# wangkenpu/rsrgan

Hardware: AMD Instinct MI355X
Metric: GAN train frames/sec (G+D step), 257-dim LPS->40-dim MFCC (higher is better)
Workload: dtype f32

## Files before the change

rsrgan_amd/csrc/capi.cpp:

```cpp
#include <cstring>
#include <exception>
#include <new>
#include <vector>

#include "model.h"

using namespace rsr;

struct rsrgan_handle_s { Model m; };

#define CHECK_H(h)                                                    \
  if (!(h)) { set_error("null handle"); return RSRGAN_ERR_INVALID; }

template <class F>
static int guard(const char* what, F&& body) {
  try {
    return body();
  } catch (const std::bad_alloc&) {
    set_error("%s: out of host memory", what);
  } catch (const std::exception& e) {
    set_error("%s: %s", what, e.what());
  } catch (...) {
    set_error("%s: unknown C++ exception", what);
  }
// ... 398 lines not shown
    float ms = 0.f;
    if (hipEventElapsedTime(&ms, m.prof_ev[2 * i], m.prof_ev[2 * i + 1]) != hipSuccess) { set_error("hipEventElapsedTime failed"); return RSRGAN_ERR_HIP; }
    us += 1e3 * ms;
  }
  *launches = m.prof_n; *total_us = us; *alg_flops = m.prof_flops;
  return RSRGAN_OK;
}
int rsrgan_profile_read_kind(rsrgan_handle h, int32_t kind, int32_t* launches, double* total_us, double* alg_flops) {
  CHECK_H(h);
  if (kind == 0) return rsrgan_profile_read(h, launches, total_us, alg_flops);
  Model& m = h->m;
  if (kind == 3 && launches && total_us && alg_flops) {
    *launches = m.prof_fdt_n; *total_us = 0.0; *alg_flops = 0.0;
    return RSRGAN_OK;
  }
  if (kind >= 4 && kind <= 8 && launches && total_us && alg_flops) {
    *launches = m.prof_cnt[kind]; *total_us = 0.0; *alg_flops = 0.0;
    return RSRGAN_OK;
  }
  if ((kind != 1 && kind != 2) || !launches || !total_us || !alg_flops) { set_error("profile_read_kind: bad argument"); return RSRGAN_ERR_INVALID; }
  std::vector<hipEvent_t>& ev = kind == 1 ? m.prof_gp_ev : m.prof_gb_ev;
  const int n = kind == 1 ? m.prof_gp_n : m.prof_gb_n;
  double us = 0.0;
  for (int i = 0; i < n; ++i) {
    if (hipEventSynchronize(ev[2 * i + 1]) != hipSuccess) { set_error("hipEventSynchronize failed"); return RSRGAN_ERR_HIP; }
    float ms = 0.f;
    if (hipEventElapsedTime(&ms, ev[2 * i], ev[2 * i + 1]) != hipSuccess) { set_error("hipEventElapsedTime failed"); return RSRGAN_ERR_HIP; }
    us += 1e3 * ms;
  }
  *launches = n; *total_us = us; *alg_flops = kind == 1 ? m.prof_gp_flops : m.prof_gb_flops;
  return RSRGAN_OK;
// ... 50 lines not shown
```

rsrgan_amd/csrc/gpersist.hip:

```cpp
#include <type_traits>

#include "kernels.h"

namespace rsr {

typedef float f32x4 __attribute__((ext_vector_type(4)));
typedef unsigned u32x4 __attribute__((ext_vector_type(4)));
typedef __attribute__((address_space(1))) unsigned gu32;
#include "dpersist_dev.h"

constexpr int GP_NR = GP_ROWS / 16;
constexpr int GP_WAVES = 12;
static_assert(GP_NR == 2, "chunk index = 2 * k-block + row tile");
constexpr int GP_NKB = 18;
constexpr int GP_KBW = 5;
constexpr int GP_SLOT = 1024;
constexpr unsigned GP_SENT = 0xFFFFFFFFu;
#ifndef GP_R1_STEPS
#define GP_R1_STEPS 3
#endif
constexpr int GP_R1 = GP_R1_STEPS;
constexpr int GP_NCH = GP_NKB * GP_NR;
constexpr unsigned GP_SC1 = 16u;
constexpr unsigned GP_VOL = 1u << 31;
// ... 851 lines not shown
      const unsigned g1 = gen + 1u;
      __hip_atomic_store(ctl + DP_CTL_GEN, g1 >= (1u << 21) ? 1u : g1, __ATOMIC_RELAXED, __HIP_MEMORY_SCOPE_AGENT);
    }
  }
}

#ifndef GP_XR_STEPS
#define GP_XR_STEPS 6
#endif
constexpr int GP_XR = GP_XR_STEPS;

template <int NT>
struct GpLdsB {
  unsigned cnt_p[GP_NR], cnt_h[GP_NR], cnt_m[GP_NR], cnt_g[GP_NR], cnt_z[GP_NR], cnt_f[GP_NR], cnt_q[GP_NR], cnt_d[GP_NR], dead, pad_[3];
  float peep[4 * NT][4];
  float car[4][2][GP_NR][64][2];
  float gs[2][GP_NR][2][64][4];
  float st[4][GP_ROWS][4 * NT];
  float pfs[GP_NR][5][16][4 * NT];
  float wpb[GP_NKB][16][4];
  float dzB[GP_NR][NT][64][4];
  float pd[4][GP_NR][NT][64];
  float wpa[GP_NKB][64][4];
  float mB[GP_NR][GP_NKB][64][4];
  float kl[8][NT][64][4];
};

__device__ __forceinline__ bool gp_poll(const GpBuf& b, unsigned so, bool son, gu32* err) {
  const unsigned long long t0 = __builtin_amdgcn_s_memrealtime();
  for (unsigned polls = 0;; ++polls) {
// ... 260 lines not shown
#pragma unroll
    for (int r = 0; r < NR; ++r)
#pragma unroll
      for (int sl = 0; sl < 2; ++sl)
        *reinterpret_cast<float2*>(&S.car[w][sl][r][lane][0]) = make_float2(L.c[((size_t)T * N + row0 + 16 * r + lr) * H + min(cell0 + 4 * (w + 4 * sl) + q, H - 1)], 0.f);
    float* const carw = &S.car[w][0][0][lane][0];
    const float* const pfc = &S.pfs[0][0][lr][4 * w + q];
    const float* const mbw = &S.mB[0][w][lane][0];
    const float* const wpw = &S.wpa[w][lane][0];
    const float* const wpv = &S.wpb[w][4 * q + (lr >> 2)][0];
    float* const pdw = &S.pd[w][0][0][lane];
    const float* const pdc = &S.pd[0][0][w][lane];
    const float* const pwc = &S.peep[4 * w + q][0];
    float* const dzw = &S.dzB[0][w][lane][0];
    float* const stc = &S.st[0][lr][4 * w + q];
    for (int s = 0; s < T; ++s) {
      const int t = T - 1 - s;
#ifdef GP_TRACE
      if (s == 0 && w == 0 && lane == 0) gp_tr[0][22] = (unsigned)__builtin_amdgcn_s_memtime();
#endif
#pragma unroll
      for (int r = 0; r < NR; ++r) {
        if (r >= nrt) continue;
        GPTSR(6 * r + 0);
        if (!gp_wait(cnt + C_M + r, 2u * ((unsigned)s + 1u), dead)) return;
        GPTSR(6 * r + 1);

        {
          f32x4 d0 = {0.f, 0.f, 0.f, 0.f}, d1 = {0.f, 0.f, 0.f, 0.f};
          __builtin_amdgcn_s_setprio(2);
// ... 33 lines not shown
            const float gi = pq[0], gj = pq[16 * CW], gf = pq[2 * 16 * CW], go = pq[3 * 16 * CW], cp = pq[4 * 16 * CW];
            const float2 cv = *reinterpret_cast<const float2*>(carw + (sl * NR + r) * 128);
            const float cc = cv.x, dcv = cv.y;
            const float tc = gp_tanh(cc);
            const float dao = dh * tc * go * (1.f - go);
            const float dcn = dcv + dh * go * (1.f - tc * tc) + dao * pw[2];
            const float daf = dcn * cp * gf * (1.f - gf);
            const float dai = dcn * gj * gi * (1.f - gi);
            const float dj = dcn * gi * (1.f - gj * gj);
            const float dcx = live ? dcn * gf + dai * pw[0] + daf * pw[1] : dcv;
            *reinterpret_cast<float2*>(carw + (sl * NR + r) * 128) = make_float2(cp, dcx);
            const f32x4 dz = {live ? dai : 0.f, live ? dj : 0.f, live ? daf : 0.f, live ? dao : 0.f};
            *reinterpret_cast<f32x4*>(dzw + (r * NT + 4 * sl) * 256) = dz;
            float* const d = stc + r * 16 * CW + sl * 16;
            d[0 * GP_ROWS * CW] = dz[0]; d[1 * GP_ROWS * CW] = dz[1]; d[2 * GP_ROWS * CW] = dz[2]; d[3 * GP_ROWS * CW] = dz[3];
          }
        }
        asm volatile("s_waitcnt vmcnt(0)" ::: "memory");
        gp_signal(cnt + C_H + r, lane);
        GPTSR(6 * r + 4);
        if (!gp_wait(cnt + C_H + r, 4u * ((unsigned)s + 1u), dead)) return;
        if (t > 0) { product(r, (int)((c1 + (unsigned)s) % GP_R1), ((c1 + (unsigned)s) / GP_R1) & 1u); gp_signal(cnt + C_Q + r, lane); }
        GPTSR(6 * r + 5);
        int ln = lane;
        asm volatile("" : "+v"(ln));
#pragma unroll
        for (int it = 0; it < (4 * 16 * NT + 255) / 256; ++it) {
          const int e = it * 256 + w * 64 + ln;
          const int cq = e % NT, pr = e / NT, row = 16 * r + (pr & 15), k = min(pr >> 4, 3);
          const float4 v = *reinterpret_cast<const float4*>(&S.st[k][row][4 * cq]);
          float* dst = L.gates + ((size_t)t * N + row0 + row) * H4 + k * H + cell0 + 4 * cq;
#ifdef GP_ABL2
          if (GP_ABL2 & 16) continue;
#endif
          if (e < 4 * 16 * NT && cell0 + 4 * cq < H) gp_stash_store(dst, v);
        }
        if (!TAG && reducer) {
          if (s > 0) gp_rearm(b1, slot1((s - 1) % GP_R1, r, jbr, 0) + (unsigned)hh * 512u, NC, w, lane);
          if (!top) gp_rearm(b3, slot1(s % GP_XR, r, jbr, 0) + (unsigned)hh * 512u, NC, w, lane);
          if (dxr && s > 0) {
            if (!gp_wait(cnt + C_D + r, (unsigned)s, dead)) return;
            gp_rearm(b3x, slot1((s - 1) % GP_XR, r, jbr, 0) + (unsigned)hh * 512u, NC, w, lane);
          }
        }
      }
    }
    if (!TAG && dxr) {
#pragma unroll
      for (int r = 0; r < NR; ++r) {
        if (r >= nrt) continue;
        if (!gp_wait(cnt + C_D + r, (unsigned)T, dead)) return;
        gp_rearm(b3x, slot1((T - 1) % GP_XR, r, jbr, 0) + (unsigned)hh * 512u, NC, w, lane);
      }
    }
#ifdef GP_TRACE
    if (w == 0) { { const int i0_ = 0, i1_ = 12; GPT_FLUSH(); } { const int i0_ = 22, i1_ = 24; GPT_FLUSH(); } }
#endif
// ... 857 lines not shown
  return gp_grid(a) <= device_cu_count();
}
__global__ void k_arm(uint4* p, size_t n16) {
  const uint4 v = {0xFFFFFFFFu, 0xFFFFFFFFu, 0xFFFFFFFFu, 0xFFFFFFFFu};
  for (size_t i = (size_t)blockIdx.x * blockDim.x + threadIdx.x; i < n16; i += (size_t)gridDim.x * blockDim.x) p[i] = v;
}
void gpersist_arm_bytes(void* p, size_t bytes, hipStream_t s) {
  hipLaunchKernelGGL(k_arm, dim3(1024), dim3(256), 0, s, (uint4*)p, bytes / 16);
}
static void gp_arm_gran2(const GPersistArgs& a, hipStream_t s) {
  const int ngr = a.N / GP_ROWS, ngl = a.ngl ? a.ngl : ngr;
  const size_t per_grp = (size_t)a.nl * a.T * GP_NCH * GP_SLOT, region = (size_t)ngr * per_grp;
  for (int rg = 0; rg < (a.res ? 2 : 1); ++rg)
    gpersist_arm_bytes((char*)a.gran2 + rg * region + (size_t)a.grp0 * per_grp, (size_t)ngl * per_grp, s);
}
size_t gpersist_gran1_bytes(const GPersistArgs& a) { return (size_t)(a.N / GP_ROWS) * a.nl * GP_R1 * GP_NCH * a.NC * GP_SLOT; }
size_t gpersist_gran2_bytes(const GPersistArgs& a) { return (size_t)(a.res ? 2 : 1) * (a.N / GP_ROWS) * a.nl * a.T * GP_NCH * GP_SLOT; }
size_t gpersist_gran3_bytes(const GPersistArgs& a) { return (size_t)(a.N / GP_ROWS) * (a.nl + 1) * GP_XR * GP_NCH * a.NC * GP_SLOT; }

void gpersist_arm(const GPersistArgs& a, hipStream_t s) {
  (void)hipMemsetAsync(a.gran1, 0xFF, gpersist_gran1_bytes(a), s);
  if (a.gran3) (void)hipMemsetAsync(a.gran3, 0xFF, gpersist_gran3_bytes(a), s);
  (void)hipMemsetAsync(a.ctl + 4, 0, 12 * sizeof(unsigned), s);
}
#ifndef GP_PROG_ONLY
#define GP_PROG_ONLY 0
#endif
void launch_glstm_fwd(const GPersistArgs& a, hipStream_t s) {
  gp_arm_gran2(a, s);
  const dim3 g(gp_grid(a)), b(GP_WAVES * 64);
// ... 97 lines not shown
```

rsrgan_amd/csrc/kernels.h:

```cpp
#pragma once
#include <hip/hip_runtime.h>
#include <stdint.h>

#include "switches.h"

namespace rsr {

constexpr int MAXJ = 8;

struct Place { int x0, nx, sb, se, nb, w; };
constexpr int JOBMAP_MAX = 768;
struct JobMap { int valid; unsigned char job[JOBMAP_MAX]; };
struct PlanItem { int ncol, nrow; double cost; int mult; };
int plan_places(int n, const PlanItem* items, Place* out);

enum { DYN_G_LR = 0, DYN_D_LR = 1, DYN_LAMBDA = 2, DYN_D_REAL = 3, DYN_D_FAKE = 4, DYN_L2 = 5, DYN_CLIP = 6,
       DYN_B1 = 7, DYN_B2 = 8, DYN_EPS = 9, DYN_EMA = 10, DYN_ADAM_LRT = 11, DYN_ADAM_LRT_D = 12, DYN_COUNT = 16 };

struct FwdGateJob {
  const float* x;
  const float* KxT;
  const float* m;
  const float* KhT;
  const float* Wsw;
// ... 150 lines not shown
  unsigned* ctl;
  float forget_bias;
  unsigned long long* gran3;
  const float* dout_top;
  int ld_dout;
  float* din0;
  int ld_din0;
  int res;
  int tags;
  int dout_trail;
  int fwd_trail;
  int ngl, grp0;
  int nrt;
  int sched;
  int carry;
};
constexpr int GP_TMAX = 2046;
bool gpersist_plan(GPersistArgs& a);
void gpersist_arm_bytes(void* p, size_t bytes, hipStream_t s);
extern thread_local int g_gemm_workers;
int gpersist_grid(const GPersistArgs& a);
int gpersist_dt_grid(const GPersistArgs& a, const DPersistArgs& d);
void launch_glstm_fwd_dt(const GPersistArgs& a, const DPersistArgs& d, hipStream_t s);
size_t dpersist_fwdt_lds_bytes();
void launch_glstm_bwd_dt(const GPersistArgs& a, const DPersistArgs& d, hipStream_t s);
size_t gpersist_lds_bytes();
int device_cu_count();
bool resident_probe(int grid, int threads, size_t lds_bytes);
size_t gpersist_gran1_bytes(const GPersistArgs& a);
size_t gpersist_gran2_bytes(const GPersistArgs& a);
// ... 62 lines not shown
                       int W, int fw, hipStream_t s,
                       float* db = nullptr );
void launch_im2col(const float* src, size_t row_stride, int ldc, int C, int S, int W, int kh, int kw, float* col, int ldk, size_t M,
                   hipStream_t s);
void launch_expand_c4(const float* src, int ld_src, int n, float* dst, size_t rows, hipStream_t s);
void launch_col2im(const float* dcol, int ldk, int C, int S, int W, int kh, int kw, float* dst, int ldc, size_t M, hipStream_t s);
struct GStateLayer { float *c, *mst; int H, P, ldP, off; };
struct GStateArgs { GStateLayer L[GP_MAXL]; int nl, SF, rows, dir; float* state; size_t slot; const int* mask; };
void launch_gstate(const GStateArgs& a, hipStream_t s);
struct ZeroList { int n; float* p[32]; unsigned len[32]; };
void launch_zero_many(const ZeroList& zl, hipStream_t s);
struct ColsumsBatch { const float* dz[4]; const float* cprev[4]; const float* ccur[4]; float* db[4]; float* dwi[4]; float* dwf[4]; float* dwo[4]; int n; };
void launch_lstm_colsums_batch(const ColsumsBatch& bt, int rows, int H, float* scratch, hipStream_t s);
void launch_lstm_colsums(const float* dz, const float* cprev, const float* ccur, float* db, float* dwi, float* dwf, float* dwo,
                         int rows, int H, float* scratch , hipStream_t s);
void launch_lrelu_bwd(const float* hval, float* d, size_t rows, int cols, int ld, float alpha, hipStream_t s);
void launch_dropout_fwd(float* y, size_t rows, int cols, int ld, unsigned long long key, unsigned thr, float keep, hipStream_t s);
void launch_dropout_bwd(const float* y, float* d, size_t rows, int cols, int ld, float keep, hipStream_t s);
void launch_colsum_tall(const float* a, int lda, float* out, int rows, int cols, float* scratch, size_t scratch_floats, hipStream_t s);

struct BnVars {
  float *beta, *gamma;
  float *mm, *mv, *rm, *rmw, *rs, *rsw;
};
constexpr int BN_STAT_ROWS = 6;
void launch_bn_forward(const float* z, int ldz, float* y, int ldy, int rows, int cols, const BnVars& v, float* stat, int ldc, bool training,
                       bool relu, float* scratch, size_t scratch_floats, hipStream_t s, int calls = 1);
void launch_bn_backward(float* dy, int ldd, const float* y, int ldy, const float* z, int ldz, int rows, int cols, const float* stat, int ldc,
                        float* dbeta, float* dgamma, bool accumulate, bool relu, float* sums, float* scratch, size_t scratch_floats,
                        hipStream_t s, int calls = 1);
// ... 48 lines not shown
```

rsrgan_amd/csrc/kernels.hip:

```cpp
#include <algorithm>
#include <cstdlib>

#include "kernels.h"

namespace rsr {

typedef float f32x4 __attribute__((ext_vector_type(4)));

__device__ __forceinline__ float sigmoid_(float x) { return 1.0f / (1.0f + expf(-x)); }

#ifdef RSR_TRACE
__device__ unsigned long long g_trace[8192 * 16];
#define TR_BEGIN() do { if (threadIdx.x == 0 && blockIdx.x < 8192) { unsigned long long* t_ = g_trace + (size_t)blockIdx.x * 16; \
    t_[0] = __builtin_amdgcn_s_memrealtime(); t_[1] = __builtin_amdgcn_s_memtime(); \
    t_[14] = __builtin_amdgcn_s_getreg(4 | (0 << 6) | (31 << 11)); t_[15] = __builtin_amdgcn_s_getreg(20 | (0 << 6) | (3 << 11)); \
    for (int i_ = 2; i_ < 14; ++i_) t_[i_] = 0; } } while (0)
#define TR_ID(ptr) do { if (threadIdx.x == 0 && blockIdx.x < 8192) g_trace[(size_t)blockIdx.x * 16 + 12] = (unsigned long long)(size_t)(ptr); } while (0)
#define TR(i) do { if (threadIdx.x == 0 && blockIdx.x < 8192) g_trace[(size_t)blockIdx.x * 16 + (i)] = __builtin_amdgcn_s_memtime(); } while (0)
#define TR_END() do { if (threadIdx.x == 0 && blockIdx.x < 8192) { g_trace[(size_t)blockIdx.x * 16 + 9] = __builtin_amdgcn_s_memtime(); \
    g_trace[(size_t)blockIdx.x * 16 + 13] = __builtin_amdgcn_s_memrealtime(); } } while (0)
#else
#define TR_BEGIN() do { } while (0)
#define TR_ID(ptr) do { } while (0)
#define TR(i) do { } while (0)
// ... 1427 lines not shown
  const int c = blockIdx.x * blockDim.x + threadIdx.x;
  if (c >= H) return;
  float s[7] = {0.f, 0.f, 0.f, 0.f, 0.f, 0.f, 0.f};
#pragma unroll 8
  for (int i = 0; i < CS_SLICES; ++i)
#pragma unroll
    for (int k = 0; k < 7; ++k) s[k] += scratch[((size_t)i * 7 + k) * H + c];
  float* db = bt.db[p];
  db[c] = s[0]; db[H + c] = s[1]; db[2 * H + c] = s[2]; db[3 * H + c] = s[3];
  bt.dwi[p][c] = s[4]; bt.dwf[p][c] = s[5]; bt.dwo[p][c] = s[6];
}
void launch_lstm_colsums_batch(const ColsumsBatch& bt, int rows, int H, float* scratch, hipStream_t s) {
  hipLaunchKernelGGL(k_lstm_colsums1_b, dim3((H + 63) / 64, CS_SLICES, bt.n), dim3(256), 0, s, bt, scratch, rows, H);
  hipLaunchKernelGGL(k_lstm_colsums2_b, dim3((H + 255) / 256, bt.n), dim3(256), 0, s, scratch, bt, H);
}
void launch_lstm_colsums(const float* dz, const float* cprev, const float* ccur, float* db, float* dwi, float* dwf, float* dwo,
                         int rows, int H, float* scratch, hipStream_t s) {
  hipLaunchKernelGGL(k_lstm_colsums1, dim3((H + 63) / 64, CS_SLICES), dim3(256), 0, s, dz, cprev, ccur, scratch, rows, H);
  hipLaunchKernelGGL(k_lstm_colsums2, dim3((H + 255) / 256), dim3(256), 0, s, scratch, db, dwi, dwf, dwo, H);
}

void launch_colsum(const float* a, int lda, const float* b, int ldb, float* out, int rows, int cols, float* scratch, hipStream_t s) {
  hipLaunchKernelGGL(k_colsum1, dim3((cols + 63) / 64, CS_SLICES), dim3(256), 0, s, a, lda, b, ldb, scratch, rows, cols);
  hipLaunchKernelGGL(k_colsum2, dim3((cols + 255) / 256), dim3(256), 0, s, scratch, out, cols);
}

__device__ __forceinline__ float block_sum_1024(float v, float* red) {
  for (int o = 32; o > 0; o >>= 1) v += __shfl_down(v, o, 64);
  const int w = threadIdx.x >> 6;
  if ((threadIdx.x & 63) == 0) red[w] = v;
// ... 358 lines not shown
```

rsrgan_amd/csrc/model.cpp:

```cpp
#include "model.h"

#include <cmath>
#include <cstdarg>
#include <cstdio>
#include <cstdlib>
#include <cstring>
#include <random>

namespace rsr {

static thread_local char g_err[512] = "";
void set_error(const char* fmt, ...) {
  va_list ap;
  va_start(ap, fmt);
  vsnprintf(g_err, sizeof(g_err), fmt, ap);
  va_end(ap);
}
const char* get_error() { return g_err; }

#define HIPC(expr)                                                                   \
  do {                                                                               \
    hipError_t e_ = (expr);                                                          \
    if (e_ != hipSuccess) {                                                          \
      set_error("%s failed: %s (%s:%d)", #expr, hipGetErrorString(e_), __FILE__, __LINE__); \
// ... 465 lines not shown
        }
        if (!gp_gran1) gp_gran1 = gp_gran2;
        if (gp_gran2 && gp_ctl) {
          HIPC(ctl_reset(gp_ctl));
          gpersist_rearm();
        } else { gp_gran1 = gp_gran2 = gp_gran3 = nullptr; gp_ctl = nullptr; }
      }
    } else if (gpersist_args(ga, gp_Tcap) && resident_probe(gpersist_grid(ga), GP_THREADS, gpersist_lds_bytes())) {
      gp_gran1 = (unsigned long long*)alloc<float>(gpersist_gran1_bytes(ga) / sizeof(float));
      gp_gran2_bytes = gpersist_gran2_bytes(ga);
      gp_gran2 = (unsigned long long*)alloc<float>(gp_gran2_bytes / sizeof(float));
      gp_ctl = (unsigned*)alloc<float>(16);
      bool bwd_ok = (gp_live & 2) != 0;
      for (auto& L : gl) bwd_ok = bwd_ok && L.P > 16;
      if (bwd_ok) gp_gran3 = (unsigned long long*)alloc<float>(gpersist_gran3_bytes(ga) / sizeof(float));
      if (gp_gran1 && gp_gran2 && gp_ctl) {
        HIPC(ctl_reset(gp_ctl));
        gpersist_rearm();
      } else { gp_gran1 = gp_gran2 = nullptr; gp_ctl = nullptr; }
    }
  }
  {
    GPersistArgs ga{};
    if (sw.trail && dp_gran && (dp_live & 2) && gp_gran1 && gp_gran3 && !gp_noproj && (gp_live & 2) && B % 32 == 0 && gpersist_args(ga, gp_Tcap))
      trail_fits = resident_probe(gpersist_grid(ga) + ((dpersist_trail_grid((int)dl.size(), B) + 7) & ~7), GP_THREADS,
                                  std::max(gpersist_lds_bytes(), dpersist_trail_lds_bytes()));
  }
  {
    lazy_sw = switches().lazy_swizzle && wavefront() && gp_gran1 && gp_gran3 && (gp_live & 3) == 3 && dp_gran && (dp_live & 3) == 3;
  }
// ... 670 lines not shown
    if (!a.res) {
      if (resi ? (R.res_in != g_ins[0] || R.res_out != g_res[l]) : (R.res_in || R.res_out)) return false;
      if (l > 0 && (R.din_accumulate || ch[l].din != ch[l - 1].dout)) return false;
    } else {
      if (R.res_in != g_ins[l] || R.res_out != g_res[l] || R.dout != ch.back().dout) return false;
      if (l > 0 ? (!R.din_accumulate || R.din != R.dout) : R.din != nullptr) return false;
    }
  }
  if (!a.res && ch[0].din && ch[0].din_accumulate) return false;
  a.dout_top = ch.back().dout; a.ld_dout = gl.back().ldP;
  if (!a.dout_top) return false;
  if (check_only) return true;
  const bool din_inside = ch[0].din && switches().gp_din0 && (gl[0].I + 15) / 16 <= (gl[0].P + 15) / 16 && gl[0].ldI % 4 == 0;
  if (din_inside) { a.din0 = ch[0].din; a.ld_din0 = gl[0].ldI; }
  a.dout_trail = gp_trail_next ? switch_now_trail_dbg() : 0;
  if (gp_phase == 2) {
  } else if (prof_on) {
    if ((size_t)(2 * prof_gb_n + 2) > prof_gb_ev.size()) {
      const size_t old = prof_gb_ev.size();
      prof_gb_ev.resize(old + 8, nullptr);
      for (size_t i = old; i < prof_gb_ev.size(); ++i) (void)hipEventCreate(&prof_gb_ev[i]);
    }
    for (size_t l = 0; l < gl.size(); ++l)
      prof_gb_flops += 2.0 * Bt * T * ((double)((l || din_inside ? gl[l].I : 0) + gl[l].P) * 4.0 * gl[l].H + (double)gl[l].H * gl[l].P);
    if (gp_trail_next) {
      for (size_t l = 0; l < dl.size(); ++l)
        prof_gb_flops += 2.0 * Bt * T * ((double)(dl[l].I + dl[l].P) * 4.0 * dl[l].H + (double)dl[l].H * dl[l].P);
      prof_gb_flops += 2.0 * Bt * T * (double)Dout * gR;
    }
    (void)hipEventRecord(prof_gb_ev[2 * prof_gb_n], s);
    glstm_bwd_groups(a, gp_trail_next ? &dt_args : nullptr, s);
    (void)hipEventRecord(prof_gb_ev[2 * prof_gb_n + 1], s);
    ++prof_gb_n;
  } else
    glstm_bwd_groups(a, gp_trail_next ? &dt_args : nullptr, s);
  if (gp_phase == 1) return true;
  auto din0 = [&](hipStream_t q) {
    if (ch[0].din && !din_inside) {
      const LayerRun& R = ch[0];
      const int H4 = 4 * R.L->H;
      gemm(R.S->gates, H4, true, R.ps->W(R.L->tK), H4, true, R.din, R.L->ldI, T * R.N, R.L->I, H4, nullptr, 0, 0.f, false, q);
    }
  };
  if (!defer_wgrads) chain_wgrads(ch, T, s, din0, pre, post);
  else { if (pre) pre(s); din0(s); if (post) post(s); }
  return true;
}

bool Model::persist_backward(Chain& ch, int T, hipStream_t s) {
  if (!dp_gran || !(dp_live & 2) || !wavefront() || ch.size() != dl.size() || ch[0].din) return false;
  DPersistArgs a{};
  a.nl = (int)ch.size(); a.N = ch[0].N; a.T = T; a.H = dl[0].H; a.len = ch[0].len;
  a.gran = dp_gran; a.ctl = dp_ctl; a.forget_bias = cfg.forget_bias;
  for (size_t l = 0; l < ch.size(); ++l) {
    const LayerRun& R = ch[l]; const LstmLayer& L = dl[l]; const LstmStash& S = d_st[l];
    if (R.L != &L || R.S != &S || R.res_in || R.res_out || R.row0 != 0 || R.Ns != R.N || R.N != a.N || !L.has_proj || L.H != a.H) return false;
    if (l > 0 && R.in != d_st[l - 1].out) return false;
    DPersistLayer& D_ = a.L[l];
    D_.K = D.W(L.tK); D_.bias = D.W(L.tb); D_.wi = D.W(L.twi); D_.wf = D.W(L.twf); D_.wo = D.W(L.two); D_.Wp = D.W(L.tWp);
    D_.gates = S.gates; D_.c = S.c; D_.h = S.h; D_.mst = S.mst; D_.out = S.out; D_.dmt = S.dmt;
// ... 82 lines not shown
  float* scr = (side && s == side) ? scratch2 : scratch;
  auto small = [&](int M, int N, int K) { const double outs = (double)M * N; return !(K >= 256 && outs >= 4.0e6) && !(K >= 2048 && outs >= 1.5e6); };
  if (check_only) { *dK_done = dK_too && small(L0.I + L0.P, H4, Rws); return small(H, L0.P, Rws); }
  if (dK_too && small(L0.I + L0.P, H4, Rws)) {
    Gemm16Batch bt{}; bt.n = (int)rs.size();
    for (int p = 0; p < bt.n; ++p) { bt.A[p] = rs[p]->in; bt.A2[p] = rs[p]->S->mst; bt.B[p] = rs[p]->S->gates; bt.C[p] = rs[p]->ps->Gd(rs[p]->L->tK); }
    launch_gemm16_batch(bt, L0.ldI, L0.ldP, L0.I, H4, H4, L0.I + L0.P, H4, Rws, false, s, ws, gemm_ws_floats);
    *dK_done = true;
  }
  if (!small(H, L0.P, Rws)) return false;
  {
    Gemm16Batch bt{}; bt.n = (int)rs.size();
    for (int p = 0; p < bt.n; ++p) { bt.A[p] = rs[p]->S->h; bt.A2[p] = nullptr; bt.B[p] = rs[p]->S->dmt; bt.C[p] = rs[p]->ps->Gd(rs[p]->L->tWp); }
    launch_gemm16_batch(bt, L0.ldH, 0, 0, L0.ldP, L0.ldP, H, L0.P, Rws, false, s, ws, gemm_ws_floats);
  }
  {
    ColsumsBatch cb{}; cb.n = (int)rs.size();
    for (int p = 0; p < cb.n; ++p) {
      const LayerRun& R = *rs[p]; const LstmLayer& L = *R.L; const ParamSet& ps = *R.ps;
      cb.dz[p] = R.S->gates; cb.cprev[p] = R.S->c; cb.ccur[p] = R.S->c + (size_t)R.N * H;
      cb.db[p] = ps.Gd(L.tb); cb.dwi[p] = ps.Gd(L.twi); cb.dwf[p] = ps.Gd(L.twf); cb.dwo[p] = ps.Gd(L.two);
    }
    launch_lstm_colsums_batch(cb, Rws, H, scr, s);
  }
  return true;
}
void Model::layer_wgrads_colsums(const LayerRun& R, int T, hipStream_t s, float* scr) {
  const LstmLayer& L = *R.L; const LstmStash& S = *R.S; const ParamSet& ps = *R.ps;
  const int H = L.H, H4 = 4 * H, Rws = T * R.N;
  (void)H4;
  launch_lstm_colsums(S.gates, S.c, S.c + (size_t)R.N * H, ps.Gd(L.tb), ps.Gd(L.twi), ps.Gd(L.twf), ps.Gd(L.two), Rws, H, scr, s);
}
void Model::layer_wgrads(const LayerRun& R, int T, hipStream_t s) {
  layer_wgrads_gemms(R, 0, T, false, s);
  layer_wgrads_colsums(R, T, s, (side && s == side) ? scratch2 : scratch);
}
void Model::chain_wgrads(Chain& ch, int T, hipStream_t s, const StreamFn& between, const StreamFn& pre, const StreamFn& post) {
  int nw = 0;
  for (auto& R : ch) nw += R.want_wgrads ? 1 : 0;
  if (!side || switches().wgrad_streams < 2 || nw < 2) {
    if (pre) pre(s);
    if (between) between(s);
    if (post) post(s);
    for (auto& R : ch)
      if (R.want_wgrads) layer_wgrads(R, T, s);
    return;
// ... 693 lines not shown
  }
  if (inl) apply_inlined |= 1;
  if (!reuse) g_fwd_valid = true;
  if (wave_bwd) {
    int bi = 0;
    if (bucketed) mark_bucket(RSRGAN_NET_G, bi++, s);
    if (cfg.g_type == RSRGAN_G_LSTM && !fcs_inside) {
      run_seg(seg_key(SEG_G_FCIN, T, kbits), s, [&]() {
        launch_lrelu_bwd(g_h0, bufA, (size_t)R, P, ldP, cfg.lrelu_alpha, s);
        gemm(x_tm, ldDin, false, bufA, ldP, false, G.Gd(g_fc_in_w), ldP, Din, P, R, nullptr, 0, 0.f, false, s);
        launch_colsum(bufA, ldP, nullptr, 0, G.Gd(g_fc_in_b), R, P, scratch, s);
      });
      if (bucketed) mark_bucket(RSRGAN_NET_G, bi++, s);
    }
    if (bucketed) {
      bool dkd = false;
      const bool gb = batch_wgrads(bw_chains[1], T, s, false, &dkd, true);
      if (gb) run_seg(seg_key(SEG_G_BATCH, T, kbits), s, [&]() { bool d_ = false; (void)batch_wgrads(bw_chains[1], T, s, false, &d_); });
      int li = 0;
      for (auto& Rr : bw_chains[1]) {
        run_seg(seg_key(SEG_G_LAYER0 + li, T, kbits), s, [&]() { if (gb) layer_wgrads_gemms(Rr, 0, T, false, s, true, false); else layer_wgrads(Rr, T, s); });
        mark_bucket(RSRGAN_NET_G, bi++, s);
        ++li;
      }
    }
  }
  if (!inl) run_seg(seg_key(SEG_G_TAIL, T, kbits), s, tail_body);
  if (want_grads) {
    if (l2_on) for (auto& bk : gbk[RSRGAN_NET_G]) bk.marked = false;
    finish_buckets(RSRGAN_NET_G, s);
    g_grads_ready = true;
  }
  if (out_losses) launch_copy_f(losses + 3, out_losses, 4, s);
  HIPC(hipGetLastError());
  return RSRGAN_OK;
}

int Model::bnl_step(const float* x, const float* labels, const int32_t* lengths, int T, float* out_losses, bool want_grads, hipStream_t s) {
  if (want_grads && cfg.cross_validation) {
// ... 71 lines not shown
```

rsrgan_amd/csrc/model.h:

```cpp
#pragma once
#include <hip/hip_runtime.h>
#include <stdint.h>
#include <string>
#include <unordered_map>
#include <functional>
#include <vector>

#include "../../include/rsrgan.h"
#include "kernels.h"

namespace rsr {

inline int pad4(int x) { return (x + 3) & ~3; }

struct TensorDesc {
  std::string name;
  int rows, cols, ld;
  int64_t off;
  int64_t dense_off;
  bool l2;
  bool trainable = true;
  bool is_vector;
  int xavier_fan_out = 0;
  float bias_init = 0.f;
// ... 142 lines not shown
  bool persist_forward_g_trail(Chain& ch, int T, hipStream_t s, const float* nf, bool check_only = false);
  bool dpipe = false;
  bool dfree_inside = false;
  bool dfree_current = false;
  int gp_phase = 0;
  hipEvent_t ev_dfree = nullptr, ev_real = nullptr;
  unsigned long long* dp_gran2 = nullptr;
  unsigned* dp_ctl2 = nullptr;
  bool persist_forward_real(int T, hipStream_t q, bool check_only = false);
  bool trail_fits = false;
  bool gp_trail_next = false;
  DPersistArgs dt_args{};
  unsigned long long *gp_gran1 = nullptr, *gp_gran2 = nullptr, *gp_gran3 = nullptr;
  unsigned* gp_ctl = nullptr;
  size_t gp_gran2_bytes = 0;
  int gp_live = sw.gpersist;
  int gp_Tcap = 0;
  float* dw_ws = nullptr; unsigned* dw_flag = nullptr; long long* dw_src = nullptr; size_t dw_stride = 0;
  bool d_partial_fresh = false;
  int dp_max_grid = 0;
  void persist_disable(int which);
  bool gp_fwd_on() const { return gp_gran1 && (gp_live & 1); }
  bool gpersist_shape(GPersistArgs& a, int T) const;
  int gp_np_nt = 0;
  bool gp_noproj = false;
  bool gpersist_args(GPersistArgs& a, int T) const;
  void gpersist_rearm();
  bool persist_forward_g(int T, hipStream_t s);
  float* g_state = nullptr;
  int g_state_sf = 0;
  bool g_carry = false;
// ... 93 lines not shown
  int apply_inlined = 0;
  void refresh_transposes(int net, hipStream_t s);
  void refresh_swizzles(int net, hipStream_t s);
  bool lazy_sw = false;

  void rnn_forward(std::vector<Chain>& chains, int T, hipStream_t s, const std::vector<int>* offsets = nullptr,
                   const std::vector<FcStage>* fcs = nullptr);
  void rnn_backward(std::vector<Chain>& chains, int T, hipStream_t s, const std::vector<int>* offsets = nullptr,
                    const std::vector<FcStage>* fcs = nullptr);
  void layer_wgrads(const LayerRun& R, int T, hipStream_t s);
  void chain_wgrads(Chain& ch, int T, hipStream_t s, const StreamFn& between, const StreamFn& pre = nullptr, const StreamFn& post = nullptr);
  void layer_wgrads_gemms(const LayerRun& R, int t0, int t1, bool accumulate, hipStream_t s, bool do_dK = true, bool do_dWp = true);
  int trail_nrt() const;
  bool batch_wgrads(Chain& ch, int T, hipStream_t s, bool dK_too, bool* dK_done, bool check_only = false);
  void layer_wgrads_colsums(const LayerRun& R, int T, hipStream_t s, float* scr);
  hipStream_t side = nullptr;
  struct GradBucket { int64_t off = 0, count = 0; hipEvent_t ev = nullptr; bool marked = false; };
  std::vector<GradBucket> gbk[2];
  bool fused_apply = false;
  bool defer_wgrads = false;
  int build_buckets();
  void mark_bucket(int net, int i, hipStream_t s);
  void finish_buckets(int net, hipStream_t s);
  bool prof_on = false;
  std::vector<hipEvent_t> prof_ev;
  int prof_n = 0;
  double prof_flops = 0.0;
  std::vector<hipEvent_t> prof_gp_ev;
  int prof_gp_n = 0;
  double prof_gp_flops = 0.0;
  std::vector<hipEvent_t> prof_gb_ev;
  int prof_gb_n = 0;
  int prof_fdt_n = 0;
  int prof_cnt[9] = {};
  double prof_gb_flops = 0.0;
  void gates_launch(const FwdGateJobs& gj, int blocks, int kb, hipStream_t s);
  int gates_blocks(int H, int N) const;
  int proj_blocks(int P, int N) const;
  int bwd_a_blocks(int H, int N) const;
  void run_bwd_b_splitk(BwdBJobs& bj, hipStream_t s);
  hipEvent_t ev_pool[16] = {};
  int ev_next = 0;
  float* gemm_ws2 = nullptr;
  float* dk_tmp = nullptr;
  size_t dk_tmp_per = 0;
  float* scratch2 = nullptr;
  bool overlap() const { return side != nullptr && (cfg.flags & RSRGAN_FLAG_OVERLAP) != 0; }
  Chain g_chain(int T);
  Chain d_chain(int N, int Ns, int row0);
// ... 32 lines not shown
```

rsrgan_amd/csrc/switches.h:

```cpp
#pragma once
#include <cstdlib>

namespace rsr {

#define RSRGAN_SWITCHES(X) \
  X(GPERSIST,       gpersist,       INT,  3,    ANY,  handle,  "persistent generator recurrences (gpersist.hip): bit 0 the forward launch, bit 1 the BPTT; 0 = the launch-per-phase wavefront") \
  X(DPERSIST,       dpersist,       INT,  3,    ANY,  handle,  "persistent discriminator recurrences (dpersist.hip): bit 0 the forward launch, bit 1 the backward launch") \
  X(DFOLD,          dfold,          BOOL, 1,    ANY,  handle,  "folded small-cell recurrence of the discriminator (one launch per step); 0 = gates + projection") \
  X(TRAIL,          trail,          INT,  1,    ANY,  handle,  "the discriminator's BPTT trailing the generator's inside one launch (k_glstm_bwd_dt); 0 = two launches") \
  X(GRAPHS,         graphs,         BOOL, 1,    ANY,  handle,  "0 = RSRGAN_FLAG_GRAPH is ignored: every segment runs eagerly") \
  X(RCED_IMPLICIT,  rced_implicit,  BOOL, 1,    ANY,  handle,  "implicit-GEMM convolution for every R-CED layer it covers; 0 = patch-matrix GEMMs everywhere") \
  X(DPIPE,          dpipe,          INT,  0,    ANY,  handle,  "D(real) of the D-run ahead on the side stream: > 0 covers labels and lengths, >= 2 a noise_real tensor too (include/rsrgan.h)") \
  X(PAD_ROWS,       pad_rows,       BOOL, 1,    ANY,  process, "pad the batch to a multiple of 32 rows so that the persistent generator recurrences apply; 0 = the caller's row count") \
  X(DW_INKERNEL,    dw_inkernel,    BOOL, 1,    ANY,  process, "the discriminator's weight gradients inside its stand-alone BPTT launch; 0 = GEMM / column-sum launches behind it") \
  X(GP_NP_BWD,      gp_np_bwd,      BOOL, 1,    ANY,  process, "persistent BPTT of an unprojected generator (8 cells per workgroup); 0 = its BPTT takes the launch path") \
  X(GP_NP_NT,       gp_np_nt,       INT,  0,    ANY,  process, "gate tiles per workgroup of the unprojected generator's launches: 2 or 4; 0 = what the resident probe admits") \
  X(GP_NOPROJ,      gp_noproj,      BOOL, 1,    ANY,  process, "persistent forward recurrence for num_proj=None generators (the single-hop form); 0 = launch path") \
  X(GP_RES,         gp_res,         BOOL, 1,    ANY,  process, "res_lstm_l and res_lstm_i inside the persistent launches (the residual sums ride the hand-offs); 0 = launch path") \
  X(GP_TAGS,        gp_tags,        BOOL, 1,    ANY,  process, "ring slots tagged with the parity of the ring pass; 0 = slots re-armed with sentinels") \
  X(GP_NRT,         gp_nrt,         BOOL, 1,    ANY,  process, "a padded generator whose real rows fit one 16-row tile skips the padding tile; 0 = both tiles run") \
  X(DP_NRT,         dp_nrt,         BOOL, 1,    ANY,  process, "the same for the discriminator's halves of the fused launches (only together with GP_NRT); 0 = the padding tile runs") \
  X(GP_SCHED,       gp_sched,       INT,  -1,   ANY,  process, "GPersistArgs::sched 0..3: off-chain work of the forward launch behind the lane's publication; -1 = 3 from 64 rows on, else 0") \
  X(GP_DIN0,        gp_din0,        BOOL, 0,    ANY,  process, "layer 0's input gradient inside k_glstm_bwd (built, bit-stable, measured slower)") \
  X(TRAIL_FWD,      trail_fwd,      BOOL, 1,    ANY,  process, "D(G(x)) trailing the generator's forward recurrence in one launch (k_glstm_fwd_dt); 0 = separate launches") \
// ... 65 lines not shown
```

Measured before the change: 1.330 million.

## Accumulate generator LSTM bias and peephole column sums inside persistent BPTT

Inside the persistent generator BPTT kernel, each lane accumulates the per-cell gate-gradient sums and the peephole products as the steps proceed, with the second cell slot kept in LDS. At the end it reduces them across lanes and writes per-group partials to a workspace. A small finalize kernel then sums over row groups and writes the bias and peephole gradients, replacing the two-pass column-sum launches that reread the stashed gates and cell states. The cost is extra registers, LDS, and arithmetic inside the latency-critical recurrence kernel, and the path can be turned off with GPERSIST bit 2.

```diff
diff --git a/rsrgan_amd/csrc/capi.cpp b/rsrgan_amd/csrc/capi.cpp
--- a/rsrgan_amd/csrc/capi.cpp
+++ b/rsrgan_amd/csrc/capi.cpp
@@ -436,7 +436,7 @@
     *launches = m.prof_fdt_n; *total_us = 0.0; *alg_flops = 0.0;
     return RSRGAN_OK;
   }
-  if (kind >= 4 && kind <= 8 && launches && total_us && alg_flops) {
+  if (kind >= 4 && kind <= 9 && launches && total_us && alg_flops) {
     *launches = m.prof_cnt[kind]; *total_us = 0.0; *alg_flops = 0.0;
     return RSRGAN_OK;
   }
diff --git a/rsrgan_amd/csrc/gpersist.hip b/rsrgan_amd/csrc/gpersist.hip
--- a/rsrgan_amd/csrc/gpersist.hip
+++ b/rsrgan_amd/csrc/gpersist.hip
@@ -889,6 +889,7 @@
 struct GpLdsB {
   unsigned cnt_p[GP_NR], cnt_h[GP_NR], cnt_m[GP_NR], cnt_g[GP_NR], cnt_z[GP_NR], cnt_f[GP_NR], cnt_q[GP_NR], cnt_d[GP_NR], dead, pad_[3];
   float peep[4 * NT][4];
+  float cs1[64][8];
   float car[4][2][GP_NR][64][2];
   float gs[2][GP_NR][2][64][4];
   float st[4][GP_ROWS][4 * NT];
@@ -1179,6 +1180,12 @@
     const float* const pwc = &S.peep[4 * w + q][0];
     float* const dzw = &S.dzB[0][w][lane][0];
     float* const stc = &S.st[0][lr][4 * w + q];
+    float cs[7];
+#pragma unroll
+    for (int k = 0; k < 7; ++k) cs[k] = 0.f;
+    auto cs1_of = [&]() { return &S.cs1[0][0] + (__builtin_amdgcn_mbcnt_hi(~0u, __builtin_amdgcn_mbcnt_lo(~0u, 0u)) << 3); };
+    float* cs1 = cs1_of();
+    if (two) { *reinterpret_cast<f32x4*>(cs1) = f32x4{0.f, 0.f, 0.f, 0.f}; *reinterpret_cast<f32x4*>(cs1 + 4) = f32x4{0.f, 0.f, 0.f, 0.f}; }
     for (int s = 0; s < T; ++s) {
       const int t = T - 1 - s;
 #ifdef GP_TRACE
@@ -1242,6 +1249,16 @@
             *reinterpret_cast<f32x4*>(dzw + (r * NT + 4 * sl) * 256) = dz;
             float* const d = stc + r * 16 * CW + sl * 16;
             d[0 * GP_ROWS * CW] = dz[0]; d[1 * GP_ROWS * CW] = dz[1]; d[2 * GP_ROWS * CW] = dz[2]; d[3 * GP_ROWS * CW] = dz[3];
+            if (sl == 0) {
+              cs[0] += dz[0]; cs[1] += dz[1]; cs[2] += dz[2]; cs[3] += dz[3];
+              cs[4] += dz[0] * cp; cs[5] += dz[2] * cp; cs[6] += dz[3] * cc;
+            } else {
+              cs1 = cs1_of();
+              f32x4 u0 = *reinterpret_cast<const f32x4*>(cs1), u1 = *reinterpret_cast<const f32x4*>(cs1 + 4);
+              u0 += dz;
+              u1[0] += dz[0] * cp; u1[1] += dz[2] * cp; u1[2] += dz[3] * cc;
+              *reinterpret_cast<f32x4*>(cs1) = u0; *reinterpret_cast<f32x4*>(cs1 + 4) = u1;
+            }
           }
         }
         asm volatile("s_waitcnt vmcnt(0)" ::: "memory");
@@ -1269,6 +1286,26 @@
           if (dxr && s > 0) {
             if (!gp_wait(cnt + C_D + r, (unsigned)s, dead)) return;
             gp_rearm(b3x, slot1((s - 1) % GP_XR, r, jbr, 0) + (unsigned)hh * 512u, NC, w, lane);
+          }
+        }
+      }
+    }
+    if (a.cs_ws) {
+      cs1 = cs1_of();
+      float* const rec = a.cs_ws + ((size_t)(grp * a.nl + l) * NC + c) * (7 * CW);
+#pragma unroll
+      for (int sl = 0; sl < 2; ++sl) {
+        if (sl == 0 || two) {
+#pragma unroll
+          for (int k = 0; k < 7; ++k) {
+            float v = sl == 0 ? cs[k] : cs1[k];
+            v += __shfl_xor(v, 1); v += __shfl_xor(v, 2); v += __shfl_xor(v, 4); v += __shfl_xor(v, 8);
+            cs[k] = v;
+          }
+          const int cl = 4 * (w + 4 * sl) + q;
+          if (lr == 0 && cell0 + cl < H) {
+#pragma unroll
+            for (int k = 0; k < 7; ++k) rec[k * CW + cl] = cs[k];
           }
         }
       }
@@ -2156,6 +2193,7 @@
   for (int rg = 0; rg < (a.res ? 2 : 1); ++rg)
     gpersist_arm_bytes((char*)a.gran2 + rg * region + (size_t)a.grp0 * per_grp, (size_t)ngl * per_grp, s);
 }
+size_t gpersist_cs_floats(int N) { return (size_t)(N / GP_ROWS) * GP_MAXL * 40 * 7 * 4 * 5; }
 size_t gpersist_gran1_bytes(const GPersistArgs& a) { return (size_t)(a.N / GP_ROWS) * a.nl * GP_R1 * GP_NCH * a.NC * GP_SLOT; }
 size_t gpersist_gran2_bytes(const GPersistArgs& a) { return (size_t)(a.res ? 2 : 1) * (a.N / GP_ROWS) * a.nl * a.T * GP_NCH * GP_SLOT; }
 size_t gpersist_gran3_bytes(const GPersistArgs& a) { return (size_t)(a.N / GP_ROWS) * (a.nl + 1) * GP_XR * GP_NCH * a.NC * GP_SLOT; }
diff --git a/rsrgan_amd/csrc/kernels.h b/rsrgan_amd/csrc/kernels.h
--- a/rsrgan_amd/csrc/kernels.h
+++ b/rsrgan_amd/csrc/kernels.h
@@ -188,6 +188,7 @@
   int nrt;
   int sched;
   int carry;
+  float* cs_ws;
 };
 constexpr int GP_TMAX = 2046;
 bool gpersist_plan(GPersistArgs& a);
@@ -280,6 +281,9 @@
 void launch_lstm_colsums_batch(const ColsumsBatch& bt, int rows, int H, float* scratch, hipStream_t s);
 void launch_lstm_colsums(const float* dz, const float* cprev, const float* ccur, float* db, float* dwi, float* dwf, float* dwo,
                          int rows, int H, float* scratch , hipStream_t s);
+struct GpColsumsFin { float* db[GP_MAXL]; float* dwi[GP_MAXL]; float* dwf[GP_MAXL]; float* dwo[GP_MAXL]; int layer[GP_MAXL]; int n; };
+void launch_gp_colsums_fin(const GpColsumsFin& f, const float* cs_ws, const unsigned* ctl, int ngr, int nl, int NC, int NT, int H, hipStream_t s);
+size_t gpersist_cs_floats(int N);
 void launch_lrelu_bwd(const float* hval, float* d, size_t rows, int cols, int ld, float alpha, hipStream_t s);
 void launch_dropout_fwd(float* y, size_t rows, int cols, int ld, unsigned long long key, unsigned thr, float keep, hipStream_t s);
 void launch_dropout_bwd(const float* y, float* d, size_t rows, int cols, int ld, float keep, hipStream_t s);
diff --git a/rsrgan_amd/csrc/kernels.hip b/rsrgan_amd/csrc/kernels.hip
--- a/rsrgan_amd/csrc/kernels.hip
+++ b/rsrgan_amd/csrc/kernels.hip
@@ -1465,6 +1465,30 @@
   hipLaunchKernelGGL(k_lstm_colsums1_b, dim3((H + 63) / 64, CS_SLICES, bt.n), dim3(256), 0, s, bt, scratch, rows, H);
   hipLaunchKernelGGL(k_lstm_colsums2_b, dim3((H + 255) / 256, bt.n), dim3(256), 0, s, scratch, bt, H);
 }
+__global__ void k_gp_colsums_fin(const float* __restrict__ ws, const unsigned* __restrict__ ctl, const GpColsumsFin f, int ngr, int nl, int NC, int CW, int H) {
+  const int p = blockIdx.y, l = f.layer[p];
+  const int c = blockIdx.x * blockDim.x + threadIdx.x;
+  if (c >= H) return;
+  const int sl = c / CW, cl = c - sl * CW;
+  float s[7];
+#pragma unroll
+  for (int k = 0; k < 7; ++k) s[k] = 0.f;
+  for (int g = 0; g < ngr; ++g) {
+    const float* rec = ws + ((size_t)(g * nl + l) * NC + sl) * 7 * CW + cl;
+#pragma unroll
+    for (int k = 0; k < 7; ++k) s[k] = g ? s[k] + rec[k * CW] : rec[k * CW];
+  }
+  if (ctl[DP_CTL_ERR] != 0) {
+#pragma unroll
+    for (int k = 0; k < 7; ++k) s[k] = __builtin_nanf("");
+  }
+  float* db = f.db[p];
+  db[c] = s[0]; db[H + c] = s[1]; db[2 * H + c] = s[2]; db[3 * H + c] = s[3];
+  f.dwi[p][c] = s[4]; f.dwf[p][c] = s[5]; f.dwo[p][c] = s[6];
+}
+void launch_gp_colsums_fin(const GpColsumsFin& f, const float* cs_ws, const unsigned* ctl, int ngr, int nl, int NC, int NT, int H, hipStream_t s) {
+  hipLaunchKernelGGL(k_gp_colsums_fin, dim3((H + 255) / 256, f.n), dim3(256), 0, s, cs_ws, ctl, f, ngr, nl, NC, 4 * NT, H);
+}
 void launch_lstm_colsums(const float* dz, const float* cprev, const float* ccur, float* db, float* dwi, float* dwf, float* dwo,
                          int rows, int H, float* scratch, hipStream_t s) {
   hipLaunchKernelGGL(k_lstm_colsums1, dim3((H + 63) / 64, CS_SLICES), dim3(256), 0, s, dz, cprev, ccur, scratch, rows, H);
diff --git a/rsrgan_amd/csrc/model.cpp b/rsrgan_amd/csrc/model.cpp
--- a/rsrgan_amd/csrc/model.cpp
+++ b/rsrgan_amd/csrc/model.cpp
@@ -503,6 +503,7 @@
       bool bwd_ok = (gp_live & 2) != 0;
       for (auto& L : gl) bwd_ok = bwd_ok && L.P > 16;
       if (bwd_ok) gp_gran3 = (unsigned long long*)alloc<float>(gpersist_gran3_bytes(ga) / sizeof(float));
+      if (gp_gran3) gp_cs_ws = alloc<float>(gpersist_cs_floats(B));
       if (gp_gran1 && gp_gran2 && gp_ctl) {
         HIPC(ctl_reset(gp_ctl));
         gpersist_rearm();
@@ -1203,6 +1204,10 @@
   const bool din_inside = ch[0].din && switches().gp_din0 && (gl[0].I + 15) / 16 <= (gl[0].P + 15) / 16 && gl[0].ldI % 4 == 0;
   if (din_inside) { a.din0 = ch[0].din; a.ld_din0 = gl[0].ldI; }
   a.dout_trail = gp_trail_next ? switch_now_trail_dbg() : 0;
+  bool cs = gp_cs_ws && gp_cs_on;
+  for (auto& R : ch) cs = cs && R.want_wgrads && R.ps == &G;
+  if (cs) a.cs_ws = gp_cs_ws;
+  if (prof_on && cs && gp_phase != 2) ++prof_cnt[9];
   if (gp_phase == 2) {
   } else if (prof_on) {
     if ((size_t)(2 * prof_gb_n + 2) > prof_gb_ev.size()) {
@@ -1231,8 +1236,10 @@
       gemm(R.S->gates, H4, true, R.ps->W(R.L->tK), H4, true, R.din, R.L->ldI, T * R.N, R.L->I, H4, nullptr, 0, 0.f, false, q);
     }
   };
+  gp_cs_fresh = cs; gp_cs_args = a;
   if (!defer_wgrads) chain_wgrads(ch, T, s, din0, pre, post);
   else { if (pre) pre(s); din0(s); if (post) post(s); }
+  gp_cs_fresh = false;
   return true;
 }
 
@@ -1345,7 +1352,8 @@
     for (int p = 0; p < bt.n; ++p) { bt.A[p] = rs[p]->S->h; bt.A2[p] = nullptr; bt.B[p] = rs[p]->S->dmt; bt.C[p] = rs[p]->ps->Gd(rs[p]->L->tWp); }
     launch_gemm16_batch(bt, L0.ldH, 0, 0, L0.ldP, L0.ldP, H, L0.P, Rws, false, s, ws, gemm_ws_floats);
   }
-  {
+  if (gp_cs_covers(*rs[0])) gp_colsums_fin(rs.data(), (int)rs.size(), s);
+  else {
     ColsumsBatch cb{}; cb.n = (int)rs.size();
     for (int p = 0; p < cb.n; ++p) {
       const LayerRun& R = *rs[p]; const LstmLayer& L = *R.L; const ParamSet& ps = *R.ps;
@@ -1360,7 +1368,18 @@
   const LstmLayer& L = *R.L; const LstmStash& S = *R.S; const ParamSet& ps = *R.ps;
   const int H = L.H, H4 = 4 * H, Rws = T * R.N;
   (void)H4;
+  if (gp_cs_covers(R)) { const LayerRun* r1 = &R; gp_colsums_fin(&r1, 1, s); return; }
   launch_lstm_colsums(S.gates, S.c, S.c + (size_t)R.N * H, ps.Gd(L.tb), ps.Gd(L.twi), ps.Gd(L.twf), ps.Gd(L.two), Rws, H, scr, s);
+}
+void Model::gp_colsums_fin(const LayerRun* const* rs, int n, hipStream_t s) {
+  const GPersistArgs& a = gp_cs_args;
+  GpColsumsFin f{}; f.n = n;
+  for (int p = 0; p < n; ++p) {
+    const LstmLayer& L = *rs[p]->L;
+    f.db[p] = G.Gd(L.tb); f.dwi[p] = G.Gd(L.twi); f.dwf[p] = G.Gd(L.twf); f.dwo[p] = G.Gd(L.two);
+    f.layer[p] = (int)(rs[p]->S - &g_st[0]);
+  }
+  launch_gp_colsums_fin(f, gp_cs_ws, gp_ctl, a.N / GP_ROWS, a.nl, a.NC, a.NT, a.H, s);
 }
 void Model::layer_wgrads(const LayerRun& R, int T, hipStream_t s) {
   layer_wgrads_gemms(R, 0, T, false, s);
@@ -2084,6 +2103,8 @@
       if (bucketed) mark_bucket(RSRGAN_NET_G, bi++, s);
     }
     if (bucketed) {
+      gp_cs_fresh = gp_cs_ws && gp_cs_on && dl[0].ldI == ldDout && persist_backward_g(bw_chains[1], T, s, true) &&
+                    gpersist_args(gp_cs_args, T);
       bool dkd = false;
       const bool gb = batch_wgrads(bw_chains[1], T, s, false, &dkd, true);
       if (gb) run_seg(seg_key(SEG_G_BATCH, T, kbits), s, [&]() { bool d_ = false; (void)batch_wgrads(bw_chains[1], T, s, false, &d_); });
@@ -2093,6 +2114,7 @@
         mark_bucket(RSRGAN_NET_G, bi++, s);
         ++li;
       }
+      gp_cs_fresh = false;
     }
   }
   if (!inl) run_seg(seg_key(SEG_G_TAIL, T, kbits), s, tail_body);
diff --git a/rsrgan_amd/csrc/model.h b/rsrgan_amd/csrc/model.h
--- a/rsrgan_amd/csrc/model.h
+++ b/rsrgan_amd/csrc/model.h
@@ -180,7 +180,8 @@
   unsigned long long *gp_gran1 = nullptr, *gp_gran2 = nullptr, *gp_gran3 = nullptr;
   unsigned* gp_ctl = nullptr;
   size_t gp_gran2_bytes = 0;
-  int gp_live = sw.gpersist;
+  int gp_live = sw.gpersist & 3;
+  bool gp_cs_on = !(sw.gpersist & 4);
   int gp_Tcap = 0;
   float* dw_ws = nullptr; unsigned* dw_flag = nullptr; long long* dw_src = nullptr; size_t dw_stride = 0;
   bool d_partial_fresh = false;
@@ -304,6 +305,11 @@
   int trail_nrt() const;
   bool batch_wgrads(Chain& ch, int T, hipStream_t s, bool dK_too, bool* dK_done, bool check_only = false);
   void layer_wgrads_colsums(const LayerRun& R, int T, hipStream_t s, float* scr);
+  float* gp_cs_ws = nullptr;
+  bool gp_cs_fresh = false;
+  GPersistArgs gp_cs_args{};
+  bool gp_cs_covers(const LayerRun& R) const { return gp_cs_fresh && R.ps == &G && !g_st.empty() && R.S >= &g_st[0] && R.S <= &g_st.back(); }
+  void gp_colsums_fin(const LayerRun* const* rs, int n, hipStream_t s);
   hipStream_t side = nullptr;
   struct GradBucket { int64_t off = 0, count = 0; hipEvent_t ev = nullptr; bool marked = false; };
   std::vector<GradBucket> gbk[2];
@@ -322,7 +328,7 @@
   std::vector<hipEvent_t> prof_gb_ev;
   int prof_gb_n = 0;
   int prof_fdt_n = 0;
-  int prof_cnt[9] = {};
+  int prof_cnt[10] = {};
   double prof_gb_flops = 0.0;
   void gates_launch(const FwdGateJobs& gj, int blocks, int kb, hipStream_t s);
   int gates_blocks(int H, int N) const;
diff --git a/rsrgan_amd/csrc/switches.h b/rsrgan_amd/csrc/switches.h
--- a/rsrgan_amd/csrc/switches.h
+++ b/rsrgan_amd/csrc/switches.h
@@ -4,7 +4,7 @@
 namespace rsr {
 
 #define RSRGAN_SWITCHES(X) \
-  X(GPERSIST,       gpersist,       INT,  3,    ANY,  handle,  "persistent generator recurrences (gpersist.hip): bit 0 the forward launch, bit 1 the BPTT; 0 = the launch-per-phase wavefront") \
+  X(GPERSIST,       gpersist,       INT,  3,    ANY,  handle,  "persistent generator recurrences (gpersist.hip): bit 0 the forward launch, bit 1 the BPTT, bit 2 (with bit 1) the column-sum launches behind the BPTT instead of its in-kernel bias / peephole sums; 0 = the launch-per-phase wavefront") \
   X(DPERSIST,       dpersist,       INT,  3,    ANY,  handle,  "persistent discriminator recurrences (dpersist.hip): bit 0 the forward launch, bit 1 the backward launch") \
   X(DFOLD,          dfold,          BOOL, 1,    ANY,  handle,  "folded small-cell recurrence of the discriminator (one launch per step); 0 = gates + projection") \
   X(TRAIL,          trail,          INT,  1,    ANY,  handle,  "the discriminator's BPTT trailing the generator's inside one launch (k_glstm_bwd_dt); 0 = two launches") \
```

Result: no change. 1.336 million, median of 6 (+0.5%).
